# lazear/sage

Measured on NVIDIA H100. Metric: spectra/sec, higher is better.
Workload: dtype f32

## Files before the change

sage_b200/csrc/kernels.cuh:

```cuda
#pragma once
#include <type_traits>

#include "device_common.cuh"
#include "glibc_log.cuh"

#ifndef SAGE_B200_RARE_NOINLINE
#define SAGE_B200_RARE_NOINLINE 0
#endif
#if SAGE_B200_RARE_NOINLINE
#define SB_RARE __noinline__
#else
#define SB_RARE __forceinline__
#endif

namespace sb {

__device__ __forceinline__ uint32_t pep_partition(const DbView& db, float x, bool le) {
    uint32_t lo = 0, hi = db.n_pep;
    if (db.pep_lut != nullptr) {
        const float t = (x - db.plut_base) * db.plut_inv_w;
        if (t == t) {
            const int c = (int)fminf(fmaxf(floorf(t), -2.0f), (float)PEP_LUT_CELLS + 2.0f);
            lo = __ldg(db.pep_lut + min(max(c - 1, 0), (int)PEP_LUT_CELLS));
            hi = __ldg(db.pep_lut + min(max(c + 2, 0), (int)PEP_LUT_CELLS));
        }
    }
    const int kx = f32_key(x);
    while (lo < hi) {
        const uint32_t mid = lo + ((hi - lo) >> 1);
        const int k = f32_key(__ldg(db.pep_mono + mid));
        if (le ? k <= kx : k < kx) lo = mid + 1; else hi = mid;
    }
    return lo;
}

__global__ void k_setup_queries(DbView db, ScorerView sc, BatchView b, uint32_t* sort_key, uint32_t* sort_val) {
    __shared__ unsigned long long s_sum[4][8];
    const uint32_t s = blockIdx.x * blockDim.x + threadIdx.x;
    unsigned long long nq = 0, nwide = 0, maxpot = 0, npepq = 0, list_need = 0, ncta = 0;
    if (s < b.n) {
    const float pmz = b.prec_mz[s];
    const uint32_t known = b.prec_charge[s];
    const float mz = __fsub_rn(pmz, PROTON);
    const bool fold = sc.wide_window || !(known != 0 && !sc.override_charge);
    uint32_t c0 = fold ? sc.min_charge : known;
    uint32_t c1 = fold ? sc.max_charge : known;
    QueryDesc* out = b.queries + (size_t)s * sc.qmax;
    uint32_t qi = 0;
    for (uint32_t z = c0; z <= c1 && qi < sc.qmax; z++) {
        const float precursor_mass = __fmul_rn(mz, (float)z);
        Tol ptol = sc.precursor_tol;
        if (sc.wide_window) {
            float lo = -2.4f, hi = 2.4f;
            if (b.iso_lo != nullptr && !isnan(b.iso_lo[s]) && !isnan(b.iso_hi[s])) { lo = b.iso_lo[s]; hi = b.iso_hi[s]; }
            ptol.kind = 2;
            ptol.lo = __fmul_rn(lo, (float)z);
            ptol.hi = __fmul_rn(hi, (float)z);
        }
        const uint32_t mfc = max_fragment_charge(sc.max_fragment_charge_opt, z);
        for (uint32_t ii = 0; ii < sc.n_iso; ii++, qi++) {
            const int iso = (sc.min_iso != sc.max_iso) ? sc.min_iso + (int)ii : 0;
            const float qmass = __fsub_rn(precursor_mass, __fmul_rn((float)iso, NEUTRON));
            float plo, phi;
            tol_bounds(ptol, qmass, plo, phi);
            const uint32_t ppl = pep_partition(db, plo, false);
            const uint32_t left = ppl == 0 ? 0 : ppl - 1;
            const uint32_t right = max(left, pep_partition(db, phi, true));
            QueryDesc q;
            q.pre_lo = left;
            q.pre_hi = right;
            q.potential = right - left + 1;
            const bool lo_ok = left < db.n_pep && __ldg(db.pep_mono + left) >= plo;
            const bool hi_ok = right < db.n_pep && __ldg(db.pep_mono + right) <= phi;
            const long long elo = (long long)left + (lo_ok ? 0 : 1);
            const long long ehi = (long long)right - (hi_ok ? 0 : 1);
            if (ehi < elo) { q.eff_lo = 1; q.eff_hi = 0; } else { q.eff_lo = (uint32_t)elo; q.eff_hi = (uint32_t)ehi; }
            q.charge = (uint8_t)z;
            q.iso = (int8_t)iso;
            q.nfc = (uint8_t)(mfc - 1);
            q.mode = q.potential > NARROW_CAP ? 2 : ((db.pep_centric_ok && q.potential <= sc.pep_cap) ? 3 : (q.potential <= WARPQ_CAP ? 4 : 1));
            out[qi] = q;
            if (q.mode != 2 && q.potential > sc.kparam) list_need += q.potential;
            if (q.mode == 4) b.counters[C_COUNT + qi] = 1ull;
            ncta += (q.mode == 1 || q.mode == 3);
            nq++;
            if (q.mode == 2) {
                nwide++;
                QueryHits h0; h0.n = 0; h0.default_run = q.potential; h0.matched_peaks = 0; h0.scored_candidates = 0;
                b.hits[(size_t)s * sc.qmax + qi] = h0;
            }
            if (q.mode == 3) npepq++;
            if (q.potential > maxpot) maxpot = q.potential;
        }
    }
    for (; qi < sc.qmax; qi++) {
        QueryDesc q = {};
        out[qi] = q;
    }
    if (sort_key) { sort_key[s] = out[0].mode ? out[0].pre_lo : 0xFFFFFFFFu; sort_val[s] = s; }
    if (nwide) {
        unsigned long long w = atomicAdd(b.counters + C_WIDE, nwide);
        for (uint32_t j = 0; j < sc.qmax; j++)
            if (out[j].mode == 2) { if (w < b.wide_cap) b.wide_items[w] = s * sc.qmax + j; w++; }
    }
    if (ncta) {
        unsigned long long w = atomicAdd(b.counters + C_NCTA, ncta);
        for (uint32_t j = 0; j < sc.qmax; j++)
            if (out[j].mode == 1 || out[j].mode == 3) b.cta_items[w++] = s * sc.qmax + j;
    }
    for (uint32_t j = 0; j < sc.qmax; j++) {
        ReplaySlot rs; rs.off = 0; rs.item = s * sc.qmax + j; rs.n_list = 0; rs.state = 1; rs.k = 0;
        b.nslots[(size_t)s * sc.qmax + j] = rs;
    }
    }
    const uint32_t lane = threadIdx.x & 31, warp = threadIdx.x >> 5;
    for (int o = 16; o > 0; o >>= 1) {
        nq += __shfl_down_sync(0xffffffffu, nq, o);
        list_need += __shfl_down_sync(0xffffffffu, list_need, o);
        npepq += __shfl_down_sync(0xffffffffu, npepq, o);
        maxpot = max(maxpot, __shfl_down_sync(0xffffffffu, maxpot, o));
    }
    if (lane == 0) { s_sum[0][warp] = nq; s_sum[1][warp] = list_need; s_sum[2][warp] = npepq; s_sum[3][warp] = maxpot; }
    __syncthreads();
    if (threadIdx.x == 0) {
        for (uint32_t w = 1; w < (blockDim.x >> 5); w++) {
            nq += s_sum[0][w]; list_need += s_sum[1][w]; npepq += s_sum[2][w]; maxpot = max(maxpot, s_sum[3][w]);
        }
        if (nq) atomicAdd(b.counters + C_QUERIES, nq);
        if (list_need) atomicAdd(b.counters + C_NLIST_NEED, list_need);
        if (npepq) atomicAdd(b.counters + C_PEPQ, npepq);
        if (maxpot) atomicMax(b.counters + C_MAXPOT, maxpot);
    }
}


__device__ __forceinline__ uint32_t block_sum_u32(uint32_t v, uint32_t* s_warp) {
    const uint32_t lane = threadIdx.x & 31, warp = threadIdx.x >> 5, nwarps = blockDim.x >> 5;
    for (int o = 16; o > 0; o >>= 1) v += __shfl_down_sync(0xffffffffu, v, o);
    __syncthreads();
    if (lane == 0) s_warp[warp] = v;
    __syncthreads();
    uint32_t t = 0;
    for (uint32_t w = 0; w < nwarps; w++) t += s_warp[w];
    __syncthreads();
    return t;
}

constexpr uint32_t LUT_CELLS = 256;
constexpr uint32_t SPEC_LUT_CELLS = 1024;
struct LutParams { float base, inv_w; };

__device__ __forceinline__ LutParams lut_params(float first, float last, uint32_t cells = LUT_CELLS) {
    LutParams L;
    L.base = first;
    const float w = (last - first) / (float)cells;
    L.inv_w = (w > 0.0f && w < 3.0e38f) ? 1.0f / w : 0.0f;
    return L;
}
__device__ __forceinline__ float lut_edge(const LutParams& L, uint32_t c) { return L.inv_w > 0.0f ? L.base + (float)c * (1.0f / L.inv_w) : L.base; }
__device__ __forceinline__ void lut_build(const float* arr, uint32_t n, const LutParams& L, uint16_t* start, uint32_t t0, uint32_t stride,
                                          uint32_t cells = LUT_CELLS) {
    for (uint32_t c = t0; c < cells; c += stride) {
        uint32_t lo = 0;
        if (c > 0 && L.inv_w > 0.0f) {
            const float e = lut_edge(L, c);
            uint32_t hi = n;
            while (lo < hi) { const uint32_t m = (lo + hi) >> 1; if (arr[m] < e) lo = m + 1; else hi = m; }
        }
        start[c] = (uint16_t)lo;
    }
}
__device__ __forceinline__ void lut_build_walk(const float* arr, uint32_t n, const LutParams& L, uint16_t* start, uint32_t t0, uint32_t stride,
                                               uint32_t cells) {
    const uint32_t per = (cells + stride - 1) / stride;
    const uint32_t c0 = t0 * per, c1 = min(cells, c0 + per);
    if (!(L.inv_w > 0.0f)) {
        for (uint32_t c = c0; c < c1; c++) start[c] = 0;
        return;
    }
    if (c0 >= c1) return;
    uint32_t i = 0;
    if (c0 > 0) {
        const float e = lut_edge(L, c0);
        uint32_t hi = n;
        while (i < hi) { const uint32_t m = (i + hi) >> 1; if (arr[m] < e) i = m + 1; else hi = m; }
    }
    start[c0] = (uint16_t)i;
    for (uint32_t c = c0 + 1; c < c1; c++) {
        const float e = lut_edge(L, c);
        while (arr[i] < e) i++;
        start[c] = (uint16_t)i;
    }
}
__device__ __forceinline__ uint32_t lut_start(const LutParams& L, const uint16_t* start, float x, uint32_t cells = LUT_CELLS) {
    const float t = (x - L.base) * L.inv_w;
    int c = t > 1.0f ? (int)fminf(t, (float)(cells - 1)) - 1 : 0;
    return start[c];
}

__device__ __forceinline__ void bucket_range(const DbView& db, float flo, float fhi, uint32_t& left, uint32_t& right) {
    if (db.bucket_lut == nullptr) {
        const int klo = f32_key(flo), khi = f32_key(fhi);
        binary_search_slice(db.n_bucket, [&](uint32_t i) { return f32_key(__ldg(db.bucket_min + i)) < klo; },
                            [&](uint32_t i) { return f32_key(__ldg(db.bucket_min + i)) <= khi; }, left, right);
        return;
    }
    const float t = (flo - db.blut_base) * db.blut_inv_w;
    const int c = t > 1.0f ? (int)fminf(t, (float)(BUCKET_LUT_CELLS - 1)) - 1 : 0;
    const uint32_t pp0 = __ldg(db.bucket_lut + c);
    uint32_t pp = pp0;
    float v = 0.0f;
    bool have = false;
    while (pp < db.n_bucket) {
        v = __ldg(db.bucket_min + pp);
        if (!(v < flo)) { have = true; break; }
        pp++;
    }
    left = pp == 0 ? 0 : pp - 1;
    uint32_t r;
    if (pp > 0 && flo <= fhi) {
        r = pp;
        if (have && v <= fhi) {
            r++;
            while (r < db.n_bucket && __ldg(db.bucket_min + r) <= fhi) r++;
        }
    } else {
        r = left;
        while (r < db.n_bucket && __ldg(db.bucket_min + r) <= fhi) r++;
    }
    right = r;
}

__device__ __forceinline__ uint32_t page_lower_bound(const uint2* slice, uint32_t lo, uint32_t hi, uint32_t key) {
    while (lo < hi) {
        const uint32_t mid = lo + ((hi - lo) >> 1);
        if (__ldg(&slice[mid].x) < key) lo = mid + 1; else hi = mid;
    }
    return lo;
}

__device__ __forceinline__ uint32_t page_lower_bound_dir(const DbView& db, uint32_t page, const uint2* slice, uint32_t pn, uint32_t key) {
    uint32_t lo = 0, hi = pn;
    if (db.page_grid != nullptr) {
        const uint32_t g = min(key >> db.grid_shift, db.grid_n - 1);
        const uint16_t* G = db.page_grid + (size_t)page * (db.grid_n + 1) + g;
        lo = __ldg(G);
        hi = (key >> db.grid_shift) >= db.grid_n ? pn : (uint32_t)__ldg(G + 1);
    }
    while (lo < hi) {
        const uint32_t mid = lo + ((hi - lo) >> 1);
        if (__ldg(&slice[mid].x) < key) lo = mid + 1; else hi = mid;
    }
    return lo;
}

__device__ __forceinline__ void index_probe(const DbView& db, const QueryDesc& q, float flo, float fhi, uint32_t* cnt32, uint32_t& matched, uint32_t& pages,
                                            uint32_t& entries) {
    uint32_t bl, br;
    bucket_range(db, flo, fhi, bl, br);
    for (uint32_t page = bl; page < br; page++) {
        const uint64_t pbase = (uint64_t)page * db.bucket_size;
        const uint64_t pend = min(pbase + db.bucket_size, db.n_frag);
        const uint2* slice = db.frag + pbase;
        const uint32_t pn = (uint32_t)(pend - pbase);
        const uint32_t pp = page_lower_bound_dir(db, page, slice, pn, q.pre_lo);
        const uint32_t il = pp == 0 ? 0 : pp - 1;
        uint32_t e = pp;
        for (; e < pn; e++) {
            const uint2 f = __ldg(&slice[e]);
            if (f.x > q.pre_hi) break;
            const float fmz = __uint_as_float(f.y);
            if (f.x >= q.eff_lo && f.x <= q.eff_hi && fmz >= flo && fmz <= fhi) {
                const uint32_t idx = f.x - q.pre_lo;
                atomicAdd(&cnt32[idx >> 1], 1u << ((idx & 1) * 16));
                matched++;
            }
        }
        pages++;
        entries += e - il;
    }
}

#ifndef SAGE_B200_WALK_SOLO
#define SAGE_B200_WALK_SOLO 8
#endif
constexpr uint32_t WALK_SOLO = SAGE_B200_WALK_SOLO;
constexpr uint32_t WALK_STEP = 2;
__device__ __forceinline__ uint32_t narrow_start_cell(const NarrowIndexView& nv, float flo) {
    const float tt = (flo - nv.base) * nv.inv_w;
    return tt > 1.0f ? (uint32_t)((int)fminf(tt, (float)(nv.cells - 1)) - 1) : 0u;
}
__device__ __forceinline__ void block_probe_warp(const NarrowIndexView& nv, const QueryDesc& q, uint32_t b0, uint32_t b1, bool act, float flo, float fhi,
                                                 uint32_t* cnt32, uint32_t& matched) {
    const uint32_t lane = threadIdx.x & 31;
    const uint32_t c = narrow_start_cell(nv, flo);
    for (uint32_t blk = b0; blk <= b1; blk++) {
        const uint32_t base = (uint32_t)__ldg(nv.blk_off + blk);
        const uint32_t cnt = (uint32_t)__ldg(nv.blk_off + blk + 1) - base;
        const float* mz = nv.mz + base;
        const uint16_t* off = nv.pep + base;
        const uint32_t pep0 = blk * nv.block;
        uint32_t e = cnt;
        if (act) {
            e = __ldg(nv.grp + (size_t)blk * (nv.cells / NARROW_GROUP) + c / NARROW_GROUP) + __ldg(nv.dir + (size_t)blk * nv.cells + c);
            for (uint32_t k = 0; k < WALK_SOLO && e < cnt; k += WALK_STEP, e += WALK_STEP) {
                float m[WALK_STEP];
                uint32_t o[WALK_STEP];
#pragma unroll
                for (uint32_t j = 0; j < WALK_STEP; j++) {
                    const bool in = e + j < cnt;
                    m[j] = in ? __ldg(mz + e + j) : __int_as_float(0x7f800000);
                    o[j] = in ? __ldg(off + e + j) : 0u;
                }
                bool stop = false;
#pragma unroll
                for (uint32_t j = 0; j < WALK_STEP; j++) {
                    stop |= m[j] > fhi;
                    const uint32_t pid = pep0 + o[j];
                    if (!stop && m[j] >= flo && pid >= q.eff_lo && pid <= q.eff_hi) {
                        const uint32_t idx = pid - q.pre_lo;
                        atomicAdd(&cnt32[idx >> 1], 1u << ((idx & 1) * 16));
                        matched++;
                    }
                }
                if (stop) { e = cnt; break; }
            }
        }
        uint32_t pend = __ballot_sync(0xffffffffu, e < cnt);
        while (pend) {
            const int src = __ffs(pend) - 1;
            pend &= pend - 1;
            const uint32_t e0 = __shfl_sync(0xffffffffu, e, src);
            const float lo_s = __shfl_sync(0xffffffffu, flo, src), hi_s = __shfl_sync(0xffffffffu, fhi, src);
            for (uint32_t pos = e0; pos < cnt; pos += 32) {
                const uint32_t i = pos + lane;
                bool stop = i >= cnt;
                if (!stop) {
                    const float fmz = __ldg(mz + i);
                    const uint32_t pid = pep0 + __ldg(off + i);
                    stop = fmz > hi_s;
                    if (!stop && fmz >= lo_s) {
                        if (pid >= q.eff_lo && pid <= q.eff_hi) {
// ... 1051 lines not shown
    __device__ __forceinline__ void matched(uint32_t index) {
        if (last == index) return;
        if (start + length == index) { length += 1; longest = max(longest, length); }
        else { start = index; length = 1; longest = max(longest, length); }
        last = index;
    }
};

struct SpecView { const float* masses; const float* intens; uint32_t np; bool use_lut; LutParams lp; const uint16_t* lut; };

__device__ SB_RARE void score_candidate_warp(const DbView& db, const ScorerView& sc, uint64_t key, const SpecView& sp, ScoreRec* out,
                                                     uint8_t* mark ) {
    const uint32_t lane = threadIdx.x & 31;
    const uint32_t pep = key_peptide(key), charge = key_charge(key);
    const uint32_t L = __ldg(db.pep_len + pep);
    const uint32_t nions = L - 1;
    const uint32_t nfc = max_fragment_charge(sc.max_fragment_charge_opt, charge) - 1;
    const float* ions = db.ions + __ldg(db.ion_off + pep);
    const uint32_t per_kind = nions * nfc, total = per_kind * db.n_kinds;
    uint32_t mb = 0, my = 0;
    float sb = 0.f, sy = 0.f, ppm = 0.f;
    Run brun = {0, 0, 0, 0}, yrun = {0, 0, 0, 0};
    for (uint32_t base = 0; base < total; base += 32) {
        const uint32_t f = base + lane;
        int pk = -1;
        float term = 0.f, inten = 0.f;
        uint32_t idx = 0;
        bool is_n = false;
        if (f < total) {
            uint32_t ki, fc;
            switch (nfc) {
                case 1: ki = f; fc = 1; break;
                case 2: ki = f >> 1; fc = (f & 1) + 1; break;
                case 3: ki = f / 3; fc = f - ki * 3 + 1; break;
                default: ki = f / nfc; fc = f - ki * nfc + 1; break;
            }
            uint32_t kind_i = ki >= nions;
            idx = ki - (kind_i ? nions : 0);
            while (idx >= nions) { idx -= nions; kind_i++; }
            is_n = (db.nterm_mask >> kind_i) & 1;
            const float ion = __ldg(ions + ki);
            const float mz = fc == 1 ? ion : (fc == 2 && fabsf(ion) >= 1e-30f) ? __fmul_rn(ion, 0.5f) : __fdiv_rn(ion, (float)fc);
            pk = sp.use_lut ? select_most_intense_peak_lut(sp.masses, sp.intens, sp.np, mz, sc.fragment_tol, sp.lp, sp.lut)
                            : select_most_intense_peak(sp.masses, sp.intens, sp.np, mz, sc.fragment_tol);
            if (pk >= 0 && mark == nullptr) {
                const float peak_mass = sp.masses[pk];
                inten = sp.intens[pk];
                term = __fdiv_rn(__fmul_rn(__fmul_rn(inten, fabsf(__fsub_rn(mz, peak_mass))), 2E6f), __fadd_rn(mz, peak_mass));
            }
        }
        if (mark != nullptr) {
            if (pk >= 0) mark[pk] = 1;
            continue;
        }
        uint32_t mask = __ballot_sync(0xffffffffu, pk >= 0);
        const uint32_t maskn = __ballot_sync(0xffffffffu, pk >= 0 && is_n);
        mb += __popc(maskn);
        my += __popc(mask & ~maskn);
        while (mask) {
            const int src = __ffs(mask) - 1;
            mask &= mask - 1;
            const float t = __shfl_sync(0xffffffffu, term, src);
            const float it = __shfl_sync(0xffffffffu, inten, src);
            const uint32_t ib = __shfl_sync(0xffffffffu, idx, src);
            ppm = __fadd_rn(ppm, t);
            if ((maskn >> src) & 1) { sb = __fadd_rn(sb, it); brun.matched(ib); }
            else { sy = __fadd_rn(sy, it); yrun.matched(ib); }
        }
    }
    if (mark == nullptr && lane == 0) {
        ScoreRec r;
        r.peptide = pep; r.charge = charge; r.iso = key_iso(key);
        r.matched_b = mb & 0xFFFF; r.matched_y = my & 0xFFFF; r.summed_b = sb; r.summed_y = sy;
        r.longest_b = brun.longest; r.longest_y = yrun.longest;
        r.hyperscore = 0.0;
        r.ppm_difference = ppm;
        r.valid = 0;
        r.plen = L;
        *out = r;
    }
}

struct FeatureOut {
    uint32_t spectrum, peptide_idx, peptide_len, rank;
    int32_t label;
    float expmass, calcmass;
    uint32_t charge;
    float rt, ims, delta_mass, isotope_error, average_ppm;
    uint32_t _pad0;
    double hyperscore, delta_next, delta_best;
    uint32_t matched_peaks, longest_b, longest_y;
    float longest_y_pct;
    uint32_t missed_cleavages;
    float matched_intensity_pct;
    uint32_t scored_candidates;
    float ms2_intensity;
    double poisson;
    uint32_t fragment_offset, fragment_count;
};
static_assert(sizeof(FeatureOut) == 128, "feature layout");
static_assert(SCORE_THREADS >= K_MAX, "k_score ranks candidates one per thread");

__device__ __forceinline__ uint32_t append_hits(uint64_t* buf, uint32_t len, uint32_t cap, const QueryHits& h, const uint64_t* keys, uint32_t kparam) {
    if (h.n) {
        for (uint32_t i = 0; i < h.n && len < cap; i++) buf[len++] = keys[i];
    } else {
        const uint32_t d = min(h.default_run, kparam);
        for (uint32_t i = 0; i < d && len < cap; i++) buf[len++] = PRESCORE_DEFAULT;
    }
    return len;
}

struct FragmentOut { int32_t kind, charge, ordinal; float intensity, mz_calculated, mz_experimental; };

struct __align__(16) CandHdr { uint32_t ion_off, base, next; uint16_t nions; uint8_t nfc, pad; };

__device__ __forceinline__ bool fast_tol_ok(float t) { const float a = fabsf(t); return t == 0.0f || (a >= 1e-9f && a <= 1e6f); }

struct CandOut { uint64_t key; uint32_t h0, hcnt; uint16_t nions; uint8_t nfc, plen; uint32_t pad; };
struct SpecMeta { unsigned long long hit_base, matched_peaks, scored; uint32_t ncand, pad; };
struct SplitOut {
    CandOut* cand;
    SpecMeta* meta;
    uint16_t* hit_k;
    float* hit_i;
    float* hit_t;
    unsigned long long hit_cap;
    struct ScoreRec* recs;
    unsigned long long* hkey;
    unsigned long long* counters;
};

__device__ __forceinline__ unsigned long long f64_sort_key(double d) {
    const unsigned long long u = (unsigned long long)__double_as_longlong(d + 0.0);
    return (u >> 63) ? ~u : (u | 0x8000000000000000ull);
}
__device__ __forceinline__ double f64_from_sort_key(unsigned long long k) {
    const unsigned long long u = (k >> 63) ? (k & 0x7FFFFFFFFFFFFFFFull) : ~k;
    return __longlong_as_double((long long)u);
}

#if SAGE_B200_PHASE_CLOCKS
__device__ unsigned long long g_phase[16];
__shared__ long long s_ph_prev;
#define PH_START() do { if (threadIdx.x == 0) s_ph_prev = clock64(); } while (0)
#define PH(i) do { if (threadIdx.x == 0) { const long long n_ = clock64(); atomicAdd(&g_phase[i], (unsigned long long)(n_ - s_ph_prev)); s_ph_prev = n_; } } while (0)
#else
#define PH_START() do {} while (0)
#define PH(i) do {} while (0)
#endif

struct ScoreTile {
    CandHdr hdr[K_MAX + 1];
    double hkey[K_MAX];
    float term[SCORE_TILE];
    float inten[SCORE_TILE];
    uint32_t mask[SCORE_TILE / 32];
    uint16_t hits[SCORE_TILE];
    uint16_t lut[SPEC_LUT_CELLS];
    uint32_t scan[SCORE_THREADS / 32];
    unsigned long long hit_base;
    uint32_t hit_room;
};

__device__ __forceinline__ uint32_t kind_index(uint32_t ki, uint32_t nions) {
    uint32_t kind = ki >= nions;
    uint32_t idx = ki - (kind ? nions : 0);
    while (idx >= nions) { idx -= nions; kind++; }
    return kind << 13 | idx;
}

__device__ __forceinline__ bool fast_task(float ion, uint32_t fc, float tlo, float thi, const SpecView& sp, const uint16_t* lut, const float* pm, float& mz,
                                          uint32_t& idx) {
    const float q3 = __fmul_rn(ion, 1.0f / 3.0f);
    const float third = __fmaf_rn(__fmaf_rn(-q3, 3.0f, ion), 1.0f / 3.0f, q3);
    mz = fc == 1 ? ion : (fc == 2 ? __fmul_rn(ion, 0.5f) : third);
    const float pl = __fmul_rn(mz, tlo), ph = __fmul_rn(mz, thi);
    const float ql = __fmul_rn(pl, 1.0f / 1000000.0f), qh = __fmul_rn(ph, 1.0f / 1000000.0f);
    const float lo = __fadd_rn(mz, __fmaf_rn(__fmaf_rn(-ql, 1000000.0f, pl), 1.0f / 1000000.0f, ql));
    const float hi = __fadd_rn(mz, __fmaf_rn(__fmaf_rn(-qh, 1000000.0f, ph), 1.0f / 1000000.0f, qh));
    const float tt = __fmul_rn(__fsub_rn(lo, sp.lp.base), sp.lp.inv_w);
    const int cc = tt > 1.0f ? (int)fminf(tt, (float)(SPEC_LUT_CELLS - 1)) - 1 : 0;
    idx = lut[cc];
    while (pm[idx] < lo) idx++;
    return pm[idx] <= hi;
}

template <bool FAST, bool SPLIT>
__device__ __forceinline__ void score_candidates_flat(const DbView& db, const ScorerView& sc, const uint64_t* cur, uint32_t ncand, const SpecView& sp,
                                                      ScoreTile& S, ScoreRec* recs, const SplitOut& so, uint32_t spec) {
    const uint32_t tid = threadIdx.x, lane = tid & 31, warp = tid >> 5, nwarps = SCORE_THREADS / 32;
    constexpr uint32_t tile = SCORE_TILE;
    uint64_t key = 0;
    uint32_t L = 0, nions = 0, nfc = 1, total = 0, ion_off = 0;
    if (tid < ncand) {
        key = cur[tid];
        const uint32_t pep = key_peptide(key);
        L = __ldg(db.pep_len + pep);
        nions = L - 1;
        nfc = max_fragment_charge(sc.max_fragment_charge_opt, key_charge(key)) - 1;
        total = nions * nfc * db.n_kinds;
        ion_off = __ldg(db.ion_off + pep);
    }
    uint32_t incl = total;
#pragma unroll
    for (int o = 1; o < 32; o <<= 1) {
        const uint32_t v = __shfl_up_sync(0xffffffffu, incl, o);
        if (lane >= (uint32_t)o) incl += v;
    }
    if (lane == 31) S.scan[warp] = incl;
    __syncthreads();
    uint32_t base = incl - total, T = 0;
#pragma unroll
    for (uint32_t w = 0; w < nwarps; w++) {
        const uint32_t x = S.scan[w];
        if (w < warp) base += x;
        T += x;
    }
    if (tid < ncand) { CandHdr h; h.ion_off = ion_off; h.base = base; h.next = base + total; h.nions = (uint16_t)nions; h.nfc = (uint8_t)nfc; h.pad = 0; S.hdr[tid] = h; }
    if (tid == 0) { CandHdr h; h.ion_off = 0; h.base = T; h.next = 0xFFFFFFFFu; h.nions = 0; h.nfc = 1; h.pad = 0; S.hdr[ncand] = h; }
    uint32_t hcnt = 0, hits_before = 0;
    if (SPLIT && tid == 0) {
        const unsigned long long hb = atomicAdd(so.counters + C_HITS, (unsigned long long)T);
        const bool room = hb + T <= so.hit_cap;
        S.hit_base = hb;
        S.hit_room = room ? 1u : 0u;
        so.meta[spec].hit_base = hb;
        if (!room) so.meta[spec].ncand = 0;
    }
    uint32_t mb = 0, my = 0;
    float sb = 0.f, sy = 0.f, ppm = 0.f;
    Run brun = {0, 0, 0, 0}, yrun = {0, 0, 0, 0};
    const float tlo = sc.fragment_tol.lo, thi = sc.fragment_tol.hi;
    const float* const pm = sp.masses;
    const float* const pi = sp.intens;
    auto generic_task = [&](const CandHdr& h, uint32_t f, uint32_t slot) -> bool {
        uint32_t ki, fc;
        switch (h.nfc) {
            case 1: ki = f; fc = 1; break;
            case 2: ki = f >> 1; fc = (f & 1) + 1; break;
            case 3: ki = f / 3; fc = f - ki * 3 + 1; break;
            default: ki = f / h.nfc; fc = f - ki * h.nfc + 1; break;
        }
        const float ion = __ldg(db.ions + h.ion_off + ki);
        const float mz = fc == 1 ? ion : (fc == 2 && fabsf(ion) >= 1e-30f) ? __fmul_rn(ion, 0.5f) : __fdiv_rn(ion, (float)fc);
        const int pk = sp.use_lut ? select_most_intense_peak_lut(pm, pi, sp.np, mz, sc.fragment_tol, sp.lp, S.lut)
                                  : select_most_intense_peak(pm, pi, sp.np, mz, sc.fragment_tol);
        if (pk < 0) return false;
        const float peak_mass = pm[pk], inten = pi[pk];
        S.term[slot] = __fdiv_rn(__fmul_rn(__fmul_rn(inten, fabsf(__fsub_rn(mz, peak_mass))), 2E6f), __fadd_rn(mz, peak_mass));
        S.inten[slot] = inten;
        return true;
    };
    for (uint32_t t0 = 0; t0 < T; t0 += tile) {
        const uint32_t tn = min(tile, T - t0);
        __syncthreads();
        PH(t0 == 0 ? 3 : 5);
        constexpr uint32_t STEP = 32 * SCORE_UNROLL;
        const uint32_t chunk = (((tn + nwarps - 1) / nwarps) + STEP - 1) & ~(STEP - 1);
        const uint32_t w_lo = min(tn, warp * chunk), w_hi = min(tn, w_lo + chunk);
        uint32_t c = 0, wcount = 0;
        CandHdr h = S.hdr[0];
        if (w_lo < w_hi) {
            const uint32_t t_first = t0 + min(w_lo + lane, w_hi - 1);
            uint32_t lo = 0, hi = ncand;
            while (hi - lo > 1) { const uint32_t mid = (lo + hi) >> 1; if (S.hdr[mid].base <= t_first) lo = mid; else hi = mid; }
            c = lo;
            h = S.hdr[c];
        }
        for (uint32_t s0 = w_lo; s0 < w_hi; s0 += STEP) {
            const uint32_t slotA = s0 + lane, slotB = slotA + 32;
            const bool inA = slotA < w_hi, inB = SCORE_UNROLL == 2 && slotB < w_hi;
            bool hitA = false, hitB = false, finalA = false, finalB = false;
            uint32_t fA = 0, fB = 0;
            CandHdr hA = h, hB = h;
            if (inA) {
                const uint32_t t = t0 + slotA;
                while (t >= h.next) { c++; h = S.hdr[c]; }
                hA = h; fA = t - h.base;
            }
            if (inB) {
                const uint32_t t = t0 + slotB;
                while (t >= h.next) { c++; h = S.hdr[c]; }
                hB = h; fB = t - h.base;
            }
            if (FAST) {
                const bool okA = inA && hA.nfc <= 3, okB = inB && hB.nfc <= 3;
                const uint32_t kiA = hA.nfc == 1 ? fA : (hA.nfc == 2 ? fA >> 1 : __umulhi(fA, 0xAAAAAAABu) >> 1);
                const uint32_t kiB = hB.nfc == 1 ? fB : (hB.nfc == 2 ? fB >> 1 : __umulhi(fB, 0xAAAAAAABu) >> 1);
                const float ionA = okA ? __ldg(db.ions + hA.ion_off + kiA) : 0.0f;
                const float ionB = okB ? __ldg(db.ions + hB.ion_off + kiB) : 0.0f;
                const bool fastA = okA && ionA >= 1.0f && ionA <= 1e20f, fastB = okB && ionB >= 1.0f && ionB <= 1e20f;
                float mzA = 0.f, mzB = 0.f;
                uint32_t idxA = 0, idxB = 0;
                if (fastA) hitA = fast_task(ionA, fA - kiA * hA.nfc + 1, tlo, thi, sp, S.lut, pm, mzA, idxA);
                if (fastB) hitB = fast_task(ionB, fB - kiB * hB.nfc + 1, tlo, thi, sp, S.lut, pm, mzB, idxB);
                if (hitA) { S.term[slotA] = mzA; S.inten[slotA] = __uint_as_float(idxA); }
                if (hitB) { S.term[slotB] = mzB; S.inten[slotB] = __uint_as_float(idxB); }
                if (inA && !fastA) hitA = finalA = generic_task(hA, fA, slotA);
                if (inB && !fastB) hitB = finalB = generic_task(hB, fB, slotB);
            } else {
                if (inA) hitA = generic_task(hA, fA, slotA);
                if (inB) hitB = generic_task(hB, fB, slotB);
            }
            const uint32_t ballA = __ballot_sync(0xffffffffu, hitA), ballB = __ballot_sync(0xffffffffu, hitB);
            if (lane == 0) { S.mask[s0 >> 5] = ballA; if (SCORE_UNROLL == 2) S.mask[(s0 >> 5) + 1] = ballB; }
            if (FAST) {
                const uint32_t lt = (1u << lane) - 1;
                if (hitA) S.hits[w_lo + wcount + __popc(ballA & lt)] = (uint16_t)(slotA | (finalA ? 0x8000u : 0u));
                wcount += __popc(ballA);
                if (SCORE_UNROLL == 2) {
                    if (hitB) S.hits[w_lo + wcount + __popc(ballB & lt)] = (uint16_t)(slotB | (finalB ? 0x8000u : 0u));
                    wcount += __popc(ballB);
                }
            }
        }
        if (FAST) {
            __syncwarp();
            for (uint32_t e = lane; e < wcount; e += 32) {
                const uint32_t ent = S.hits[w_lo + e];
                if (ent & 0x8000u) continue;
                const uint32_t slot = ent;
                const float mz = S.term[slot];
                uint32_t idx = __float_as_uint(S.inten[slot]);
                const float ph = __fmul_rn(mz, thi), qh = __fmul_rn(ph, 1.0f / 1000000.0f);
                const float hi = __fadd_rn(mz, __fmaf_rn(__fmaf_rn(-qh, 1000000.0f, ph), 1.0f / 1000000.0f, qh));
                int best = -1;
                float max_int = 0.0f;
                float m;
                do {
                    const float it = pi[idx];
                    if (it >= max_int) { max_int = it; best = (int)idx; }
                    m = pm[++idx];
                } while (m <= hi);
                if (best >= 0) {
                    const float peak_mass = pm[best];
                    S.term[slot] = __fdiv_rn(__fmul_rn(__fmul_rn(max_int, fabsf(__fsub_rn(mz, peak_mass))), 2E6f), __fadd_rn(mz, peak_mass));
                    S.inten[slot] = max_int;
                } else {
                    atomicAnd(&S.mask[slot >> 5], ~(1u << (slot & 31)));
                }
            }
        }
        __syncthreads();
        PH(4);
        if (SPLIT) {
            const uint32_t nwords = (tn + 31) >> 5;
            const uint32_t mw = lane < nwords ? S.mask[lane] : 0u;
            uint32_t incl = (uint32_t)__popc(mw);
#pragma unroll
            for (int o = 1; o < 32; o <<= 1) {
                const uint32_t v = __shfl_up_sync(0xffffffffu, incl, o);
                if (lane >= (uint32_t)o) incl += v;
            }
            const uint32_t pre = incl - (uint32_t)__popc(mw), tile_total = __shfl_sync(0xffffffffu, incl, 31);
            const uint32_t word = tid >> 2, q8 = (tid & 3) * 8;
            const uint32_t wm = word < nwords ? S.mask[word] : 0u;
            const uint32_t p = __shfl_sync(0xffffffffu, pre, word & 31);
            uint32_t m8 = (wm >> q8) & 0xFFu;
            const bool room = S.hit_room != 0;
            while (m8) {
                const uint32_t bit = q8 + (uint32_t)__ffs(m8) - 1;
                m8 &= m8 - 1;
                const uint32_t slot = (word << 5) + bit, t = t0 + slot;
                uint32_t lo = 0, hi = ncand;
                while (hi - lo > 1) { const uint32_t mid = (lo + hi) >> 1; if (S.hdr[mid].base <= t) lo = mid; else hi = mid; }
                while (t >= S.hdr[lo].next) lo++;
                const CandHdr hh = S.hdr[lo];
                const uint32_t f = t - hh.base;
                const uint32_t ki = hh.nfc == 1 ? f : (hh.nfc == 2 ? f >> 1 : f / hh.nfc);
                if (room) {
                    const unsigned long long g = S.hit_base + hits_before + p + (uint32_t)__popc(wm & ((1u << bit) - 1u));
                    so.hit_k[g] = (uint16_t)kind_index(ki, hh.nions);
                    so.hit_i[g] = S.inten[slot];
                    so.hit_t[g] = S.term[slot];
                }
            }
            if (tid < ncand && total) {
                const uint32_t a = max(base, t0), b = min(base + total, t0 + tn);
                if (a < b) {
                    const uint32_t sa = a - t0, se = b - t0 - 1;
                    for (uint32_t w = sa >> 5; w <= se >> 5; w++) {
                        uint32_t m = S.mask[w];
                        if (w == sa >> 5) m &= 0xffffffffu << (sa & 31);
                        if (w == se >> 5) m &= 0xffffffffu >> (31 - (se & 31));
                        hcnt += (uint32_t)__popc(m);
                    }
                }
            }
            hits_before += tile_total;
            continue;
        }
        if (tid < ncand && total) {
            const uint32_t a = max(base, t0), b = min(base + total, t0 + tn);
            if (a < b) {
                const uint32_t sa = a - t0, se = b - t0 - 1;
                for (uint32_t w = sa >> 5; w <= se >> 5; w++) {
                    uint32_t m = S.mask[w];
                    if (w == sa >> 5) m &= 0xffffffffu << (sa & 31);
                    if (w == se >> 5) m &= 0xffffffffu >> (31 - (se & 31));
                    while (m) {
                        const uint32_t slot = (w << 5) + (uint32_t)__ffs(m) - 1;
                        m &= m - 1;
                        const uint32_t f = t0 + slot - base;
                        uint32_t ki;
                        switch (nfc) {
                            case 1: ki = f; break;
                            case 2: ki = f >> 1; break;
                            case 3: ki = f / 3; break;
                            default: ki = f / nfc; break;
                        }
                        uint32_t kind_i = ki >= nions;
                        uint32_t idx = ki - (kind_i ? nions : 0);
                        while (idx >= nions) { idx -= nions; kind_i++; }
                        const float it = S.inten[slot];
                        ppm = __fadd_rn(ppm, S.term[slot]);
                        if ((db.nterm_mask >> kind_i) & 1) { mb++; sb = __fadd_rn(sb, it); brun.matched(idx); }
                        else { my++; sy = __fadd_rn(sy, it); yrun.matched(idx); }
                    }
                }
            }
        }
    }
    if (SPLIT) {
        uint32_t inc2 = hcnt;
#pragma unroll
        for (int o = 1; o < 32; o <<= 1) {
            const uint32_t v = __shfl_up_sync(0xffffffffu, inc2, o);
            if (lane >= (uint32_t)o) inc2 += v;
        }
        __syncthreads();
        if (lane == 31) S.scan[warp] = inc2;
        __syncthreads();
        uint32_t h0 = inc2 - hcnt;
#pragma unroll
        for (uint32_t w = 0; w < nwarps; w++) if (w < warp) h0 += S.scan[w];
        if (tid < ncand) {
            CandOut co;
            co.key = key; co.h0 = h0; co.hcnt = hcnt; co.nions = (uint16_t)nions; co.nfc = (uint8_t)nfc; co.plen = (uint8_t)L; co.pad = 0;
            so.cand[(size_t)spec * sc.kparam + tid] = co;
        }
        return;
    }
    if (tid < ncand) {
        ScoreRec r;
        r.peptide = key_peptide(key); r.charge = key_charge(key); r.iso = key_iso(key);
        r.matched_b = mb & 0xFFFF; r.matched_y = my & 0xFFFF; r.summed_b = sb; r.summed_y = sy;
        r.longest_b = brun.longest; r.longest_y = yrun.longest;
        r.hyperscore = hyperscore_of(sc, r.matched_b, r.matched_y, sb, sy);
        r.ppm_difference = __fdiv_rn(ppm, __fadd_rn(sb, sy));
        r.valid = ((r.matched_b + r.matched_y) & 0xFFFF) >= sc.min_matched_peaks;
        r.plen = L;
        recs[tid] = r;
        S.hkey[tid] = r.valid ? r.hyperscore : -INFINITY;
    }
}

__device__ SB_RARE void annotate_candidate_warp(const DbView& db, const ScorerView& sc, uint32_t pep, uint32_t charge, const SpecView& sp,
                                                        FragmentOut* out, uint32_t cap_left) {
    const uint32_t lane = threadIdx.x & 31;
    const uint32_t L = __ldg(db.pep_len + pep);
    const uint32_t nions = L - 1;
    const uint32_t nfc = max_fragment_charge(sc.max_fragment_charge_opt, charge) - 1;
    const float* ions = db.ions + __ldg(db.ion_off + pep);
    const uint32_t total = nions * nfc * db.n_kinds;
    uint32_t written = 0;
    for (uint32_t base = 0; base < total; base += 32) {
        const uint32_t f = base + lane;
        int pk = -1;
        float mz = 0.f;
        uint32_t idx = 0, kind_i = 0, fc = 1;
        if (f < total) {
            const uint32_t ki = f / nfc;
            fc = f - ki * nfc + 1;
            idx = ki;
            while (idx >= nions) { idx -= nions; kind_i++; }
            mz = __fdiv_rn(__ldg(ions + ki), (float)fc);
            pk = sp.use_lut ? select_most_intense_peak_lut(sp.masses, sp.intens, sp.np, mz, sc.fragment_tol, sp.lp, sp.lut)
                            : select_most_intense_peak(sp.masses, sp.intens, sp.np, mz, sc.fragment_tol);
        }
        const uint32_t ball = __ballot_sync(0xffffffffu, pk >= 0);
        if (pk >= 0) {
            const uint32_t pos = written + __popc(ball & ((1u << lane) - 1));
            if (pos < cap_left) {
                const bool is_n = (db.nterm_mask >> kind_i) & 1;
                FragmentOut o;
                o.kind = db.kinds[kind_i];
                o.charge = (int32_t)fc;
                o.ordinal = is_n ? (int32_t)idx + 1 : (int32_t)(L == 0 ? 0 : L - 1) - (int32_t)idx;
                o.intensity = sp.intens[pk];
                o.mz_calculated = __fadd_rn(mz, PROTON);
                o.mz_experimental = __fadd_rn(sp.masses[pk], PROTON);
                out[pos] = o;
            }
        }
        written += __popc(ball);
    }
}

__device__ __forceinline__ bool spectrum_lut_setup(const float* masses , uint32_t np, uint16_t* lut, LutParams& lp) {
    bool bad = np == 0 || np >= 65536;
    for (uint32_t i = threadIdx.x; i < np; i += blockDim.x) {
        const float m = masses[i];
        bad |= !(m > 0.0f) || (i > 0 && !(m >= masses[i - 1]));
    }
    if (__syncthreads_or(bad)) return false;
    lp = lut_params(masses[0], masses[np - 1], SPEC_LUT_CELLS);
    lut_build_walk(masses, np, lp, lut, threadIdx.x, blockDim.x, SPEC_LUT_CELLS);
    __syncthreads();
    return true;
}

template <bool SPLIT>
__global__ void __launch_bounds__(SCORE_THREADS, SPLIT ? SCORE_MIN_CTAS_SPLIT : SCORE_MIN_CTAS) k_score(DbView db, ScorerView sc, BatchView b, FeatureOut* features, uint32_t* counts, uint32_t pmax,
                                                         uint64_t* dbg_keys , uint32_t* dbg_meta, FragmentOut* frag_out ,
                                                         unsigned long long frag_cap, uint32_t quick_mode ,
                                                         uint8_t* keep , SplitOut so) {
    extern __shared__ __align__(16) unsigned char smem_raw[];
    float* masses_raw = reinterpret_cast<float*>(smem_raw);
    float* intens_raw = masses_raw + pmax + 4;
    uint64_t* cur = reinterpret_cast<uint64_t*>(intens_raw + pmax + 4);
    uint64_t* tot = cur + sc.lcap;
    ScoreRec* recs = reinterpret_cast<ScoreRec*>(tot + sc.lcap);
    uint32_t* order = reinterpret_cast<uint32_t*>(recs + sc.kparam);
    uint8_t* mark = reinterpret_cast<uint8_t*>(order + sc.kparam);
    __shared__ __align__(16) ScoreTile S;
    uint16_t* const lut = S.lut;
    __shared__ uint32_t s_ntot, s_ncand, s_np, s_nvalid;
    __shared__ unsigned long long s_matched_peaks, s_scored;
    __shared__ float s_tic;

    const uint32_t s = b.order ? b.order[blockIdx.x] : blockIdx.x, tid = threadIdx.x, lane = tid & 31, warp = tid >> 5, nwarps = SCORE_THREADS / 32;
    PH_START();
    const uint32_t p0 = b.peak_off[s];
    uint32_t np = b.peak_off[s + 1] - p0;
    __shared__ __align__(8) uint64_t s_bar;
    const uint32_t a0 = p0 & ~3u, head = p0 - a0;
    const uint32_t bytes = ((head + np) * 4 + 15) & ~15u;
    float* masses = masses_raw + head;
    float* intens = intens_raw + head;
    if (tid == 0) {
        mbar_init(&s_bar, 1);
        if (np) {
            mbar_arrive_expect_tx(&s_bar, 2 * bytes);
            bulk_copy_g2s(masses_raw, b.masses + a0, bytes, &s_bar);
            bulk_copy_g2s(intens_raw, b.intens + a0, bytes, &s_bar);
        }
    }

    const QueryDesc* qd = b.queries + (size_t)s * sc.qmax;
    const QueryHits* qh = b.hits + (size_t)s * sc.qmax;
    const uint64_t* qk = b.hit_keys + (size_t)s * sc.qmax * sc.kparam;
    const bool iso_fold = sc.min_iso != sc.max_iso;
    const bool single = !iso_fold && (sc.qmax == 1 || qd[1].mode == 0) && qd[0].mode != 0;
    if (single) {
        const QueryHits h = qh[0];
        const uint32_t n = h.n ? h.n : min(h.default_run, sc.kparam);
        for (uint32_t i = tid; i < n; i += SCORE_THREADS) tot[i] = h.n ? qk[i] : PRESCORE_DEFAULT;
        __syncthreads();
        if (warp == 0) {
            uint32_t w = 0;
            for (uint32_t base = 0; base < n; base += 32) {
                const uint32_t i = base + lane;
                const uint64_t k = i < n ? tot[i] : PRESCORE_DEFAULT;
                const bool keep = i < n && key_peptide(k) != 0xFFFFFFFFu;
                const uint32_t ball = __ballot_sync(0xffffffffu, keep);
                if (keep) cur[w + __popc(ball & ((1u << lane) - 1))] = k;
                w += __popc(ball);
            }
            if (lane == 0) { s_ntot = n; s_ncand = w; s_matched_peaks = h.matched_peaks; s_scored = h.scored_candidates; s_np = np; s_tic = b.tic[s]; }
        }
    } else if (tid == 0) {
        unsigned long long mp = 0, scd = 0;
        uint32_t ntot = 0;
        uint32_t nq = 0;
        while (nq < sc.qmax && qd[nq].mode != 0) nq++;
        const uint32_t nch = sc.n_iso ? nq / sc.n_iso : 0;
        for (uint32_t ci = 0; ci < nch; ci++) {
            uint32_t ncur = 0;
            for (uint32_t ii = 0; ii < sc.n_iso; ii++) {
                const uint32_t qi = ci * sc.n_iso + ii;
                mp += qh[qi].matched_peaks;
                scd += qh[qi].scored_candidates;
                ncur = append_hits(cur, ncur, sc.lcap, qh[qi], qk + (size_t)qi * sc.kparam, sc.kparam);
            }
            if (iso_fold) {
                const uint32_t k = min(ncur, sc.kparam);
                bounded_min_heapify_seq(cur, ncur, k);
                ncur = k;
            }
            for (uint32_t i = 0; i < ncur && ntot < sc.lcap; i++) tot[ntot++] = cur[i];
        }
        {
            const uint32_t k = min(ntot, sc.kparam);
            bounded_min_heapify_seq(tot, ntot, k);
            ntot = k;
        }
        s_ntot = ntot;
        s_matched_peaks = mp;
        s_scored = scd;
        uint32_t nc = 0;
        for (uint32_t i = 0; i < ntot; i++)
            if (key_peptide(tot[i]) != 0xFFFFFFFFu) cur[nc++] = tot[i];
        s_ncand = nc;
        s_np = np;
        s_tic = b.tic[s];
    }
    __syncthreads();
    PH(0);
    if (dbg_keys != nullptr) {
        for (uint32_t i = tid; i < s_ntot; i += SCORE_THREADS) dbg_keys[(size_t)s * sc.kparam + i] = tot[i];
        if (tid == 0) { dbg_meta[s * 4 + 0] = s_ntot; dbg_meta[s * 4 + 1] = (uint32_t)s_matched_peaks; dbg_meta[s * 4 + 2] = (uint32_t)s_scored; }
    }
    if (np) mbar_wait(&s_bar, 0);
    PH(1);
    if (tid == 0) masses[np] = INFINITY;
    const uint32_t ncand = s_ncand;
    if (SPLIT && tid == 0) {
        SpecMeta m;
        m.hit_base = 0; m.matched_peaks = s_matched_peaks; m.scored = s_scored; m.ncand = ncand; m.pad = 0;
        so.meta[s] = m;
    }
    const bool lists_fit = b.counters[C_NLIST_NEED] <= b.nlist_cap && b.counters[C_WIDE] <= (unsigned long long)b.wide_cap;
    if (quick_mode != 0 && !lists_fit) return;
    if (quick_mode == 1) {
        for (uint32_t i = tid; i < ncand; i += SCORE_THREADS) keep[key_peptide(cur[i])] = 1;
        return;
    }
    const float mzp = __fsub_rn(b.prec_mz[s], PROTON);
    const double lambda = (double)s_matched_peaks / (double)s_scored;
    const uint32_t rounds = sc.chimera ? sc.report_psms : 1;
    const uint32_t per_round = sc.chimera ? 1 : sc.report_psms;
    uint32_t nout = 0;
    SpecView sv;
    sv.masses = masses; sv.intens = intens; sv.lut = lut;
    for (uint32_t round = 0; round < rounds && ncand; round++) {
        np = s_np;
        sv.np = np;
        sv.use_lut = spectrum_lut_setup(masses, np, lut, sv.lp);
        PH(2);
        if (tid == 0) s_nvalid = 0;
        if (sv.use_lut && sc.score_fast && sc.fragment_tol.kind == 0 && fast_tol_ok(sc.fragment_tol.lo) && fast_tol_ok(sc.fragment_tol.hi))
            score_candidates_flat<true, SPLIT>(db, sc, cur, ncand, sv, S, recs, so, s);
        else
            score_candidates_flat<false, SPLIT>(db, sc, cur, ncand, sv, S, recs, so, s);
        if (SPLIT) return;
        __syncthreads();
        PH(5);
        if (quick_mode == 2) {
            if (tid < ncand && recs[tid].valid) {
                const uint32_t pme = recs[tid].peptide;
                uint32_t pos = 0;
                for (uint32_t j = 0; j < ncand; j++) {
                    if (!recs[j].valid) continue;
                    const uint32_t pj = recs[j].peptide;
                    pos += (pj > pme) || (pj == pme && j < tid);
                }
                if (pos < sc.report_psms) keep[pme] = 1;
            }
            return;
        }
// ... 647 lines not shown
```

Before: 24.73 million.

## Record slot-to-candidate map in shared memory and replace binary searches with ballots

The scoring kernel now writes each slot's candidate index into a byte array that shares storage with hkey, so the hit-emission loop reads it directly instead of binary-searching the candidate headers for every hit. The per-warp starting candidate is found with a ballot/popcount over all headers rather than a per-lane binary search. The LUT build walk takes the thread stride as a template constant and hoists the cell-width reciprocal, and split-mode output now takes nions/nfc/plen from the header instead of per-thread registers. The union depends on hkey being unused during the split path, and plen is now derived as nions+1, which may not match the previous value in every case.

Result: faster. 26.07 million (median of 6 runs) (+5.4%).

```diff
diff --git a/sage_b200/csrc/kernels.cuh b/sage_b200/csrc/kernels.cuh
--- a/sage_b200/csrc/kernels.cuh
+++ b/sage_b200/csrc/kernels.cuh
@@ -170,24 +170,25 @@
         start[c] = (uint16_t)lo;
     }
 }
-__device__ __forceinline__ void lut_build_walk(const float* arr, uint32_t n, const LutParams& L, uint16_t* start, uint32_t t0, uint32_t stride,
-                                               uint32_t cells) {
-    const uint32_t per = (cells + stride - 1) / stride;
+template <uint32_t STRIDE>
+__device__ __forceinline__ void lut_build_walk(const float* arr, uint32_t n, const LutParams& L, uint16_t* start, uint32_t t0, uint32_t cells) {
+    const uint32_t per = (cells + STRIDE - 1) / STRIDE;
     const uint32_t c0 = t0 * per, c1 = min(cells, c0 + per);
     if (!(L.inv_w > 0.0f)) {
         for (uint32_t c = c0; c < c1; c++) start[c] = 0;
         return;
     }
     if (c0 >= c1) return;
+    const float w = 1.0f / L.inv_w;
     uint32_t i = 0;
     if (c0 > 0) {
-        const float e = lut_edge(L, c0);
+        const float e = L.base + (float)c0 * w;
         uint32_t hi = n;
         while (i < hi) { const uint32_t m = (i + hi) >> 1; if (arr[m] < e) i = m + 1; else hi = m; }
     }
     start[c0] = (uint16_t)i;
     for (uint32_t c = c0 + 1; c < c1; c++) {
-        const float e = lut_edge(L, c);
+        const float e = L.base + (float)c * w;
         while (arr[i] < e) i++;
         start[c] = (uint16_t)i;
     }
@@ -1545,7 +1546,10 @@
 
 struct ScoreTile {
     CandHdr hdr[K_MAX + 1];
-    double hkey[K_MAX];
+    union {
+        double hkey[K_MAX];
+        uint8_t cand[SCORE_TILE];
+    };
     float term[SCORE_TILE];
     float inten[SCORE_TILE];
     uint32_t mask[SCORE_TILE / 32];
@@ -1555,6 +1559,7 @@
     unsigned long long hit_base;
     uint32_t hit_room;
 };
+static_assert(SCORE_TILE <= sizeof(double) * K_MAX && K_MAX <= 255, "the slot -> candidate bytes fit in hkey's bytes and hold a candidate index");
 
 __device__ __forceinline__ uint32_t kind_index(uint32_t ki, uint32_t nions) {
     uint32_t kind = ki >= nions;
@@ -1653,14 +1658,15 @@
         const uint32_t chunk = (((tn + nwarps - 1) / nwarps) + STEP - 1) & ~(STEP - 1);
         const uint32_t w_lo = min(tn, warp * chunk), w_hi = min(tn, w_lo + chunk);
         uint32_t c = 0, wcount = 0;
-        CandHdr h = S.hdr[0];
         if (w_lo < w_hi) {
-            const uint32_t t_first = t0 + min(w_lo + lane, w_hi - 1);
-            uint32_t lo = 0, hi = ncand;
-            while (hi - lo > 1) { const uint32_t mid = (lo + hi) >> 1; if (S.hdr[mid].base <= t_first) lo = mid; else hi = mid; }
-            c = lo;
-            h = S.hdr[c];
-        }
+            const uint32_t t_first = t0 + w_lo;
+            uint32_t n_le = 0;
+#pragma unroll
+            for (uint32_t k = 0; k < (uint32_t)K_MAX; k += 32)
+                n_le += (uint32_t)__popc(__ballot_sync(0xffffffffu, k + lane < ncand && S.hdr[k + lane].base <= t_first));
+            c = n_le - 1;
+        }
+        CandHdr h = S.hdr[c];
         for (uint32_t s0 = w_lo; s0 < w_hi; s0 += STEP) {
             const uint32_t slotA = s0 + lane, slotB = slotA + 32;
             const bool inA = slotA < w_hi, inB = SCORE_UNROLL == 2 && slotB < w_hi;
@@ -1671,11 +1677,13 @@
                 const uint32_t t = t0 + slotA;
                 while (t >= h.next) { c++; h = S.hdr[c]; }
                 hA = h; fA = t - h.base;
+                if (SPLIT) S.cand[slotA] = (uint8_t)c;
             }
             if (inB) {
                 const uint32_t t = t0 + slotB;
                 while (t >= h.next) { c++; h = S.hdr[c]; }
                 hB = h; fB = t - h.base;
+                if (SPLIT) S.cand[slotB] = (uint8_t)c;
             }
             if (FAST) {
                 const bool okA = inA && hA.nfc <= 3, okB = inB && hB.nfc <= 3;
@@ -1755,12 +1763,9 @@
             while (m8) {
                 const uint32_t bit = q8 + (uint32_t)__ffs(m8) - 1;
                 m8 &= m8 - 1;
-                const uint32_t slot = (word << 5) + bit, t = t0 + slot;
-                uint32_t lo = 0, hi = ncand;
-                while (hi - lo > 1) { const uint32_t mid = (lo + hi) >> 1; if (S.hdr[mid].base <= t) lo = mid; else hi = mid; }
-                while (t >= S.hdr[lo].next) lo++;
-                const CandHdr hh = S.hdr[lo];
-                const uint32_t f = t - hh.base;
+                const uint32_t slot = (word << 5) + bit;
+                const CandHdr hh = S.hdr[S.cand[slot]];
+                const uint32_t f = t0 + slot - hh.base;
                 const uint32_t ki = hh.nfc == 1 ? f : (hh.nfc == 2 ? f >> 1 : f / hh.nfc);
                 if (room) {
                     const unsigned long long g = S.hit_base + hits_before + p + (uint32_t)__popc(wm & ((1u << bit) - 1u));
@@ -1829,8 +1834,9 @@
 #pragma unroll
         for (uint32_t w = 0; w < nwarps; w++) if (w < warp) h0 += S.scan[w];
         if (tid < ncand) {
+            const CandHdr h = S.hdr[tid];
             CandOut co;
-            co.key = key; co.h0 = h0; co.hcnt = hcnt; co.nions = (uint16_t)nions; co.nfc = (uint8_t)nfc; co.plen = (uint8_t)L; co.pad = 0;
+            co.key = cur[tid]; co.h0 = h0; co.hcnt = hcnt; co.nions = h.nions; co.nfc = h.nfc; co.plen = (uint8_t)(h.nions + 1); co.pad = 0;
             so.cand[(size_t)spec * sc.kparam + tid] = co;
         }
         return;
@@ -1893,13 +1899,13 @@
 
 __device__ __forceinline__ bool spectrum_lut_setup(const float* masses , uint32_t np, uint16_t* lut, LutParams& lp) {
     bool bad = np == 0 || np >= 65536;
-    for (uint32_t i = threadIdx.x; i < np; i += blockDim.x) {
+    for (uint32_t i = threadIdx.x; i < np; i += SCORE_THREADS) {
         const float m = masses[i];
         bad |= !(m > 0.0f) || (i > 0 && !(m >= masses[i - 1]));
     }
     if (__syncthreads_or(bad)) return false;
     lp = lut_params(masses[0], masses[np - 1], SPEC_LUT_CELLS);
-    lut_build_walk(masses, np, lp, lut, threadIdx.x, blockDim.x, SPEC_LUT_CELLS);
+    lut_build_walk<SCORE_THREADS>(masses, np, lp, lut, threadIdx.x, SPEC_LUT_CELLS);
     __syncthreads();
     return true;
 }
```
